# facebookresearch/habitat-lab

Hardware: AMD Instinct MI355X
Metric: env-steps/sec (SPS) PointNav RGB-D 256x256, 64 envs x 128 rollout (higher is better)
Workload: dtype f32; 1 GPU; PointNav SimpleCNN+GRU, 64 envs x 128 steps, 256x256 RGB-D synthetic; envs_per_gpu=64, rollout_steps=128, ppo_epoch=4, num_mini_batch=4, parallelism=dp1

## Files before the change

### habitat-lab_amd/csrc/gemm_ops.hip

```cpp
#include "igemm.h"
#include "igemm_dma.h"
#include "igemm_dma_wgrad.h"
#include "igemm_bf3.h"
#include "igemm_bf3_ws.h"
#include "dense_bf3.h"
#include "obs_conv_bf3.h"
#include "obs_conv_bf3_ws.h"
#include "obs_conv_patch.h"
#include "wgrad3x3_bf3.h"
#include "conv2_fwd_strip.h"
#include "conv2_dgrad_strip.h"
#include "conv3_dgrad_strip.h"
#include "obs_wgrad_bf3.h"
#include "obs_wgrad_strip.h"
#include "conv_patch_bf3.h"
#include "wgrad3x3_patch.h"
#include "prob_build.h"
#include <stdlib.h>

#include <atomic>

#include "../../include/habitat_amd.h"

namespace hab {
// ... 84 lines not shown

static bool patch3x3_wanted(const ConvDesc& d, int M) { return matrix_path_on(MP_PATCH3X3) && d.stride == 1 && d.KH == 3 && d.KW == 3 && M > 64; }
static PatchGeom patch3x3_geom(const float* in, int Hi, int Wi, int Ci, int Ho, int Wo, int off, int flip) {
    PatchGeom gq{};
    gq.in = in; gq.Hi = Hi; gq.Wi = Wi; gq.Ci = Ci; gq.Ho = Ho; gq.Wo = Wo; gq.KH = 3; gq.KW = 3;
    gq.off_h = off; gq.off_w = off; gq.flip = flip;
    return gq;
}

int conv_fwd(const ConvDesc& d, const float* x, const float* wf, const float* bias, float* y, int relu, float* ws,
             size_t ws_floats, hipStream_t stream) {
    ConvFwdProb p;
    HAB_TRY(build(p, d, x, wf, bias, y, relu));
    if (matrix_path_on(MP_CONV2_FWD | MP_RC))
        HAB_TRY_FORM(conv2_fwd_strip(p, ws, ws_floats, stream));
    if (patch3x3_wanted(d, p.M))
        HAB_TRY_FORM(conv_patch_bf3_dispatch(p, patch3x3_geom(x, d.H, d.W, d.C, p.g.Ho, p.g.Wo, -d.pad, 0), ws, ws_floats, stream));
    return run_igemm(p, ws, ws_floats, stream);
}
int64_t obs_conv_weight_image_floats() { return ((int64_t)OCP_W_ELEMS + 1) / 2 + 4; }
int obs_conv_weight_image(const float* wf, int Cout, int KH, int KW, int C, void* img, hipStream_t stream) {
    return obs_conv_patch_weight_image(wf, Cout, KH, KW, C, reinterpret_cast<unsigned short*>(img), stream);
}
int obs_conv_fwd(const ConvDesc& d, const ObsView& obs, const float* wf, const float* bias, float* y, int relu, float* ws,
                 size_t ws_floats, hipStream_t stream, const void* wimg) {
    ObsConvFwdProb p;
    HAB_TRY(build(p, d, obs, wf, bias, y, relu));
    if (matrix_path_on(MP_OBS_PATCH | MP_OBS) && p.quad)
        HAB_TRY_FORM(obs_conv_patch_launch(p, ws, ws_floats, stream, reinterpret_cast<const unsigned short*>(wimg)));
    if (matrix_path_on(MP_WS | MP_OBS) && p.quad && p.M > 64)
        HAB_TRY_FORM(obs_conv_bf3_ws_launch(p, ws, ws_floats, stream));
    if (matrix_path_on(MP_OBS) && p.quad && p.M > 64)
        HAB_TRY_FORM(obs_conv_bf3_launch<2>(p, ws, ws_floats, stream));
    return run_igemm(p, ws, ws_floats, stream);
}
__global__ void dgrad_empty_class_kernel(ConvDgradProb p) {
    const long long total = (long long)p.g.B * p.Hc * p.Wc * p.N;
    for (long long e = (long long)blockIdx.x * blockDim.x + threadIdx.x; e < total; e += (long long)gridDim.x * blockDim.x)
        p.store((int)(e / p.N), (int)(e % p.N), 0.f);
}

static int choose_conv_dgrad(const ConvDesc& d, const float* dy, const float* wd, const float* mask, const float* add, const float* dx) {
    if (!matrix_path_on(MP_CONV2_DGRAD | MP_RC)) return HAB_CONV_DGRAD_FORM_GENERAL;
    if (conv2_dgrad_strip_serves(d, dy, wd, mask, add, dx)) return HAB_CONV_DGRAD_FORM_CONV2_STRIP;
    if (conv3_dgrad_strip_serves(d, dy, wd, mask, add, dx)) return HAB_CONV_DGRAD_FORM_CONV3_STRIP;
    return HAB_CONV_DGRAD_FORM_GENERAL;
}
int conv_dgrad(const ConvDesc& d, const float* dy, const float* wd, const float* mask, const float* add, float* dx,
               float* ws, size_t ws_floats, hipStream_t stream) {
    const int form = choose_conv_dgrad(d, dy, wd, mask, add, dx);
    if (form == HAB_CONV_DGRAD_FORM_CONV2_STRIP) HAB_TRY_FORM(conv2_dgrad_strip(d, dy, wd, mask, add, dx, stream));
    if (form == HAB_CONV_DGRAD_FORM_CONV3_STRIP) HAB_TRY_FORM(conv3_dgrad_strip(d, dy, wd, mask, add, dx, stream));
// ... 271 lines not shown
    ConvDesc d;
    d.B = B; d.H = H; d.W = W; d.C = C; d.Cout = Cout; d.KH = KH; d.KW = KW; d.stride = stride; d.pad = pad;
    return d;
}
static ObsView mkobs(const uint8_t* rgb, const float* depth, const int* rows, int H, int W) {
    ObsView o;
    o.rgb = rgb; o.depth = depth; o.rows = rows; o.H = H; o.W = W; o.C = (rgb ? 3 : 0) + (depth ? 1 : 0);
    return o;
}

extern "C" int hab_conv2d_fwd(const float* x, const float* w_fwd, const float* bias, float* y, int B, int H, int W, int C,
                              int Cout, int KH, int KW, int stride, int pad, int relu, float* ws, size_t ws_floats,
                              hipStream_t stream) {
    if (!x || !w_fwd || !y) return HAB_ERR_ARG;
    return conv_fwd(mk(B, H, W, C, Cout, KH, KW, stride, pad), x, w_fwd, bias, y, relu, ws, ws_floats, stream);
}
extern "C" int hab_obs_conv2d_fwd(const uint8_t* rgb, const float* depth, const int* rows, const float* w_fwd,
                                  const float* bias, float* y, int B, int H, int W, int Cout, int KH, int KW, int stride,
                                  int pad, int relu, float* ws, size_t ws_floats, hipStream_t stream) {
    if ((!rgb && !depth) || !w_fwd || !y) return HAB_ERR_ARG;
    ObsView o = mkobs(rgb, depth, rows, H, W);
    return obs_conv_fwd(mk(B, H, W, o.C, Cout, KH, KW, stride, pad), o, w_fwd, bias, y, relu, ws, ws_floats, stream);
}
extern "C" int hab_conv2d_dgrad(const float* dy, const float* w_dgrad, const float* relu_mask, const float* add, float* dx,
                                int B, int H, int W, int C, int Cout, int KH, int KW, int stride, int pad, float* ws,
                                size_t ws_floats, hipStream_t stream) {
    if (!dy || !w_dgrad || !dx) return HAB_ERR_ARG;
    return conv_dgrad(mk(B, H, W, C, Cout, KH, KW, stride, pad), dy, w_dgrad, relu_mask, add, dx, ws, ws_floats, stream);
}
extern "C" int hab_conv2d_dgrad_form(const float* dy, const float* w_dgrad, const float* relu_mask, const float* add, float* dx,
                                     int B, int H, int W, int C, int Cout, int KH, int KW, int stride, int pad, const float* ws,
                                     size_t ws_floats) {
    (void)ws; (void)ws_floats;
    if (!dy || !w_dgrad || !dx) return HAB_ERR_ARG;
    const ConvDesc d = mk(B, H, W, C, Cout, KH, KW, stride, pad);
    const int r = check_conv(d);
    if (r != HAB_OK) return r;
    return choose_conv_dgrad(d, dy, w_dgrad, relu_mask, add, dx);
}
extern "C" int hab_conv2d_wgrad(const float* x, const float* dy, float* dw_oihw, float* dbias, int B, int H, int W, int C, int Cout,
                                int KH, int KW, int stride, int pad, float* ws, size_t ws_floats, hipStream_t stream) {
    if (!x || !dy || !dw_oihw) return HAB_ERR_ARG;
    return conv_wgrad(mk(B, H, W, C, Cout, KH, KW, stride, pad), x, dy, dw_oihw, dbias, ws, ws_floats, stream);
}
extern "C" int hab_obs_conv2d_wgrad(const uint8_t* rgb, const float* depth, const int* rows, const float* dy, float* dw_oihw,
                                    float* dbias, int B, int H, int W, int Cout, int KH, int KW, int stride, int pad, float* ws,
// ... 47 lines not shown
```

### habitat-lab_amd/csrc/obs_conv_patch.h

```cpp
#pragma once
#include <utility>

#include "igemm_bf3.h"

namespace hab {

constexpr int OCP_TH = 4;
constexpr int OCP_R = 4 * OCP_TH + 4;
constexpr int OCP_KP = 256 + 8;
constexpr int OCP_DP = 64 + 8;

constexpr int OCP_W_ELEMS = 3 * 32 * OCP_KP + 2 * 32 * OCP_DP;
__global__ void obs_patch_split_weights(const float* __restrict__ w, int N, unsigned short* __restrict__ img) {
    const int e = blockIdx.x * blockDim.x + threadIdx.x;
    if (e >= 32 * 256) return;
    const int n = e >> 8, k = e & 255, c = k & 3;
    float v = n < N ? w[(size_t)n * 256 + k] : 0.f;
    if (c < 3) v *= HAB_RCP255;
    unsigned h1, h2, h3;
    bf3_split(v, h1, h2, h3);
    img[(0 * 32 + n) * OCP_KP + k] = (unsigned short)h1;
    img[(1 * 32 + n) * OCP_KP + k] = (unsigned short)h2;
    img[(2 * 32 + n) * OCP_KP + k] = (unsigned short)h3;
    if (c == 3) {
        unsigned short* d = img + 3 * 32 * OCP_KP;
        const int kd = k >> 2;
        d[(0 * 32 + n) * OCP_DP + kd] = (unsigned short)h1;
        d[(1 * 32 + n) * OCP_DP + kd] = (unsigned short)h2;
    }
    if (k < 8) {
        img[(0 * 32 + n) * OCP_KP + 256 + k] = 0; img[(1 * 32 + n) * OCP_KP + 256 + k] = 0; img[(2 * 32 + n) * OCP_KP + 256 + k] = 0;
        unsigned short* d = img + 3 * 32 * OCP_KP;
        d[(0 * 32 + n) * OCP_DP + 64 + k] = 0; d[(1 * 32 + n) * OCP_DP + 64 + k] = 0;
    }
}

template <class F, int... Is>
__device__ __forceinline__ void ocp_static_for_impl(F& f, std::integer_sequence<int, Is...>) { (f(std::integral_constant<int, Is>()), ...); }
template <int N, class F>
__device__ __forceinline__ void ocp_static_for(F& f) { ocp_static_for_impl(f, std::make_integer_sequence<int, N>()); }

struct ObsPatchGeom {
    int W, H, Ho, Wo, tiles_per_img, ntiles;
    int units;
    int patch_elems;
};

template <int UPT>
__global__ void __launch_bounds__(512) obs_conv_patch_kernel(const ObsConvFwdProb p, const ObsPatchGeom gq, const unsigned short* __restrict__ wimg,
                                                              const int sign_schedule, const int ablate) {
    using P = ObsConvFwdProb;
    static_assert(EpiV4<P>::value, "transposed-accumulator epilogue");
    extern __shared__ __attribute__((aligned(16))) unsigned short smem16[];
    const int W = gq.W;
    const int t = threadIdx.x;
    const int lane = t & 63, wave = __builtin_amdgcn_readfirstlane(t >> 6), group = wave >> 2, gw = wave & 3, tg = t & 255;
    const int li = lane & 31, hi = lane >> 5;
    unsigned short* W12 = smem16;
    unsigned short* WD1 = W12 + 2 * 32 * OCP_KP;
    float* biasL = reinterpret_cast<float*>(WD1 + 32 * OCP_DP);
    unsigned short* P0 = WD1 + 32 * OCP_DP + 64 + group * gq.patch_elems;
    unsigned short* P1 = P0 + OCP_R * W * 4;
    unsigned short* P2 = P1 + OCP_R * W;

    for (int i = t; i < 2 * 32 * OCP_KP / 8; i += 512) reinterpret_cast<u32x4*>(W12)[i] = reinterpret_cast<const u32x4*>(wimg)[i];
    for (int i = t; i < 32 * OCP_DP / 8; i += 512) reinterpret_cast<u32x4*>(WD1)[i] = reinterpret_cast<const u32x4*>(wimg + 3 * 32 * OCP_KP)[i];
    if (t < 32) biasL[t] = (p.bias && t < p.N) ? p.bias[t] : 0.f;
    bf16x8 w3f[8][2], wd2f[4];
    {
        const unsigned short* w3 = wimg + 2 * 32 * OCP_KP + li * OCP_KP + hi * 8;
        const unsigned short* wd = wimg + 3 * 32 * OCP_KP + li * OCP_DP + hi * 8;
#pragma unroll
        for (int kh = 0; kh < 8; ++kh)
#pragma unroll
            for (int s = 0; s < 2; ++s) w3f[kh][s] = *reinterpret_cast<const bf16x8*>(w3 + kh * 32 + s * 16);
#pragma unroll
        for (int j = 0; j < 4; ++j) wd2f[j] = *reinterpret_cast<const bf16x8*>(wd + 32 * OCP_DP + j * 16);
    }

    auto tile_of = [&](int vb) {
        const int q = gq.ntiles >> 3, r = gq.ntiles & 7, xcd = vb & 7, idx = vb >> 3;
        return (xcd < r ? xcd * (q + 1) : r * (q + 1) + (xcd - r) * q) + idx;
    };

    struct Rgb12 { uint32_t d0, d1, d2; };
    Rgb12 rg[UPT];
    f32x4 dp[UPT];
    const int qpr = W >> 2;
    auto tile_base = [&](int tile, int& y0) {
        const int img = tile / gq.tiles_per_img;
        y0 = 4 * (tile - img * gq.tiles_per_img) * OCP_TH;
        return (size_t)p.obs.srow(img) * gq.H;
    };
    auto unit_pix = [&](size_t frame, int y0, int j, bool& ok) {
        const int u = tg + 256 * j;
        const int r = u / qpr, x4 = u - r * qpr;
        const int y = y0 + r;
        ok = (u < gq.units) & (y < gq.H);
        return (frame + (ok ? y : 0)) * W + 4 * (ok ? x4 : 0);
    };
    auto fetch_depth = [&](int tile) {
        if (ablate & 1) return;
        int y0;
        const size_t frame = tile_base(tile, y0);
#pragma unroll
        for (int j = 0; j < UPT; ++j) {
            bool ok;
            const size_t pix = unit_pix(frame, y0, j, ok);
            dp[j] = ld4(p.obs.depth + pix);
            if (!ok) dp[j] = zero4();
        }
    };
    auto fetch_rgb = [&](int tile) {
        if (ablate & 1) return;
        int y0;
        const size_t frame = tile_base(tile, y0);
#pragma unroll
        for (int j = 0; j < UPT; ++j) {
            bool ok;
            const size_t pix = unit_pix(frame, y0, j, ok);
            rg[j] = *reinterpret_cast<const Rgb12*>(p.obs.rgb + pix * 3);
            if (!ok) { rg[j].d0 = 0; rg[j].d1 = 0; rg[j].d2 = 0; }
        }
    };
    auto stage = [&]() {
        if (ablate & 8) return;
#pragma unroll
        for (int j = 0; j < UPT; ++j) {
            const int u = tg + 256 * j;
            if (u >= gq.units) continue;
            const unsigned d[3] = {rg[j].d0, rg[j].d1, rg[j].d2};
            unsigned f[12];
#pragma unroll
            for (int e = 0; e < 12; ++e) f[e] = __float_as_uint((float)((d[e >> 2] >> (8 * (e & 3))) & 0xffu));
            unsigned a1, a2, a3, b1, b2, b3;
            bf3_split2(dp[j][0], dp[j][1], a1, a2, a3);
            bf3_split2(dp[j][2], dp[j][3], b1, b2, b3);
            u32x4 lo, hi4;
            lo[0] = bf3_pack(f[0], f[1]);  lo[1] = bf3_pack(f[2], a1 << 16);
            lo[2] = bf3_pack(f[3], f[4]);  lo[3] = bf3_pack(f[5], a1 & 0xffff0000u);
            hi4[0] = bf3_pack(f[6], f[7]); hi4[1] = bf3_pack(f[8], b1 << 16);
            hi4[2] = bf3_pack(f[9], f[10]); hi4[3] = bf3_pack(f[11], b1 & 0xffff0000u);
            unsigned short* dst = P0 + (size_t)u * 16;
            *reinterpret_cast<u32x4*>(dst) = lo;
            *reinterpret_cast<u32x4*>(dst + 8) = hi4;
            u32x2 r1, r2;
            r1[0] = a2; r1[1] = b2; r2[0] = a3; r2[1] = b3;
            *reinterpret_cast<u32x2*>(P1 + (size_t)u * 4) = r1;
            *reinterpret_cast<u32x2*>(P2 + (size_t)u * 4) = r2;
        }
    };

    const int a_px0 = (4 * gw) * W + 4 * li;
    f32x16 acc[2];
    bf16x8 fr[2][5];
    auto load_step = [&](auto stc) {
        constexpr int st = decltype(stc)::value, set = st & 1;
        if constexpr (st < 4) {
#pragma unroll
            for (int i = 0; i < 2; ++i) {
                const int px = a_px0 + (2 * st + hi) * W + 128 * i;
                u32x4 v1, v2;
                const u32x2 l1 = *reinterpret_cast<const u32x2*>(P1 + px), h1 = *reinterpret_cast<const u32x2*>(P1 + px + 4);
                const u32x2 l2 = *reinterpret_cast<const u32x2*>(P2 + px), h2 = *reinterpret_cast<const u32x2*>(P2 + px + 4);
                v1[0] = l1[0]; v1[1] = l1[1]; v1[2] = h1[0]; v1[3] = h1[1];
                v2[0] = l2[0]; v2[1] = l2[1]; v2[2] = h2[0]; v2[3] = h2[1];
                fr[set][i] = __builtin_bit_cast(bf16x8, v1);
                fr[set][2 + i] = __builtin_bit_cast(bf16x8, v2);
            }
            fr[set][4] = *reinterpret_cast<const bf16x8*>(WD1 + li * OCP_DP + (2 * st + hi) * 8);
        } else {
            constexpr int kh = (st - 4) >> 1, s_ = (st - 4) & 1;
#pragma unroll
            for (int i = 0; i < 2; ++i)
                fr[set][i] = *reinterpret_cast<const bf16x8*>(P0 + (size_t)(a_px0 + kh * W + 128 * i) * 4 + (2 * s_ + hi) * 8);
#pragma unroll
            for (int pl = 0; pl < 2; ++pl)
                fr[set][2 + pl] = *reinterpret_cast<const bf16x8*>(W12 + (pl * 32 + li) * OCP_KP + kh * 32 + s_ * 16 + hi * 8);
        }
    };
    auto flip = [&](bf16x8 f, const unsigned sgn) {
        u32x4 v = __builtin_bit_cast(u32x4, f);
        v[0] ^= sgn; v[1] ^= sgn; v[2] ^= sgn; v[3] ^= sgn;
        return __builtin_bit_cast(bf16x8, v);
    };
    auto mma_step = [&](auto stc, const unsigned sgn) {
        constexpr int st = decltype(stc)::value, set = st & 1;
        if constexpr (st < 4) {
            const bf16x8 a1[2] = {flip(fr[set][0], sgn), flip(fr[set][1], sgn)}, a2[2] = {flip(fr[set][2], sgn), flip(fr[set][3], sgn)};
            const bf16x8 wd1 = fr[set][4];
#pragma unroll
            for (int i = 0; i < 2; ++i) acc[i] = __builtin_amdgcn_mfma_f32_32x32x16_bf16(wd1, a2[i], acc[i], 0, 0, 0);
#pragma unroll
            for (int i = 0; i < 2; ++i) acc[i] = __builtin_amdgcn_mfma_f32_32x32x16_bf16(wd2f[st], a1[i], acc[i], 0, 0, 0);
#pragma unroll
            for (int i = 0; i < 2; ++i) acc[i] = __builtin_amdgcn_mfma_f32_32x32x16_bf16(wd1, a1[i], acc[i], 0, 0, 0);
        } else {
            constexpr int kh = (st - 4) >> 1, s_ = (st - 4) & 1;
            const bf16x8 a[2] = {flip(fr[set][0], sgn), flip(fr[set][1], sgn)};
#pragma unroll
            for (int i = 0; i < 2; ++i) acc[i] = __builtin_amdgcn_mfma_f32_32x32x16_bf16(w3f[kh][s_], a[i], acc[i], 0, 0, 0);
#pragma unroll
            for (int i = 0; i < 2; ++i) acc[i] = __builtin_amdgcn_mfma_f32_32x32x16_bf16(fr[set][3], a[i], acc[i], 0, 0, 0);
#pragma unroll
            for (int i = 0; i < 2; ++i) acc[i] = __builtin_amdgcn_mfma_f32_32x32x16_bf16(fr[set][2], a[i], acc[i], 0, 0, 0);
        }
    };
    auto matrix_phase = [&](const unsigned sgn) {
#pragma unroll
        for (int i = 0; i < 2; ++i)
#pragma unroll
            for (int v = 0; v < 16; ++v) acc[i][v] = 0.0f;
        if (ablate & 2) return;
        load_step(std::integral_constant<int, 0>());
        auto body = [&](auto stc) {
            constexpr int st = decltype(stc)::value;
            if constexpr (st + 1 < 20) load_step(std::integral_constant<int, st + 1>());
            mma_step(stc, sgn);
        };
        ocp_static_for<20>(body);
    };
    auto store_tile = [&](int tile, bool neg) {
        if ((ablate & 4) && acc[0][0] != 12345.f) return;
        const int img = tile / gq.tiles_per_img, ho = (tile - img * gq.tiles_per_img) * OCP_TH + gw;
        if (ho >= gq.Ho) return;
#pragma unroll
        for (int i = 0; i < 2; ++i) {
            const int wo = 32 * i + li;
            if (wo >= gq.Wo) continue;
            const size_t base = ((size_t)(img * gq.Ho + ho) * gq.Wo + wo) * p.N;
#pragma unroll
            for (int g = 0; g < 4; ++g) {
                const int n = 8 * g + 4 * hi;
                if (n + 3 >= p.N) continue;
                f32x4 v;
                v[0] = acc[i][4 * g]; v[1] = acc[i][4 * g + 1]; v[2] = acc[i][4 * g + 2]; v[3] = acc[i][4 * g + 3];
                if (neg) { v[0] = -v[0]; v[1] = -v[1]; v[2] = -v[2]; v[3] = -v[3]; }
                v += *reinterpret_cast<const f32x4*>(biasL + n);
                if (p.relu) { v[0] = fmaxf(v[0], 0.f); v[1] = fmaxf(v[1], 0.f); v[2] = fmaxf(v[2], 0.f); v[3] = fmaxf(v[3], 0.f); }
                if (p.y) *reinterpret_cast<f32x4*>(p.y + base + n) = v;
            }
        }
    };

    const int vstep = 2 * gridDim.x;
    const int vb0 = blockIdx.x + group * gridDim.x;
    const int n_mine = vb0 < gq.ntiles ? (gq.ntiles - vb0 + vstep - 1) / vstep : 0;
    const int n_first = (int)blockIdx.x < gq.ntiles ? (gq.ntiles - (int)blockIdx.x + vstep - 1) / vstep : 0;
    if (n_first == 0) return;
    if (n_mine > 0) { fetch_depth(tile_of(vb0)); if (group == 0) fetch_rgb(tile_of(vb0)); }
    if (group == 0) stage();
    __syncthreads();
    for (int pI = 0; pI <= 2 * n_first; ++pI) {
        if ((pI & 1) == group) {
            const int k = pI >> 1;
            if (k < n_mine) {
                if (k + 1 < n_mine) fetch_depth(tile_of(vb0 + (k + 1) * vstep));
                const int tile = tile_of(vb0 + k * vstep);
                matrix_phase((sign_schedule && (tile & 1)) ? 0x80008000u : 0u);
            }
        } else {
            const int kd = (pI - 1 - group) / 2;
            const int ks = (pI + 1 - group) / 2;
            if (ks < n_mine) {
                fetch_rgb(tile_of(vb0 + ks * vstep));
                stage();
            }
            if (pI >= 1 + group && kd < n_mine) {
                const int tile_d = tile_of(vb0 + kd * vstep);
                store_tile(tile_d, sign_schedule && (tile_d & 1));
            }
        }
        __syncthreads();
    }
}

inline int obs_conv_patch_weight_image(const float* w_packed, int N, int KH, int KW, int C, unsigned short* img, hipStream_t stream) {
    if (KH != 8 || KW != 8 || C != 4 || N > 32 || (N & 3) || !w_packed || !img || (reinterpret_cast<uintptr_t>(img) & 15)) return HAB_NOT_APPLICABLE;
    obs_patch_split_weights<<<32, 256, 0, stream>>>(w_packed, N, img);
    HAB_LAUNCH_CHECK();
    return HAB_OK;
}

inline int obs_conv_patch_launch(const ObsConvFwdProb& p, float* ws, size_t ws_floats, hipStream_t stream, const unsigned short* wimg_cached = nullptr) {
    const ConvGeom& g = p.g;
    if (!p.quad || g.KH != 8 || g.KW != 8 || g.stride != 4 || g.pad != 0 || p.N > 32 || (p.N & 3) || p.K != 256 || g.W > 256 || (g.W & 3) || g.Wo > 64 ||
        g.Wo < 1 || p.M <= 0)
        return HAB_NOT_APPLICABLE;
    if (!wimg_cached && (!ws || ws_floats * 4 < (size_t)OCP_W_ELEMS * 2 || (reinterpret_cast<uintptr_t>(ws) & 15))) return HAB_NOT_APPLICABLE;
    if (reinterpret_cast<uintptr_t>(wimg_cached) & 15) return HAB_NOT_APPLICABLE;
    ObsPatchGeom gq;
    gq.W = g.W; gq.H = g.H; gq.Ho = g.Ho; gq.Wo = g.Wo;
    gq.tiles_per_img = cdiv(g.Ho, OCP_TH);
    gq.ntiles = g.B * gq.tiles_per_img;
    gq.units = OCP_R * (g.W >> 2);
    if (cdiv(gq.units, 256) > 5) return HAB_NOT_APPLICABLE;
    gq.patch_elems = OCP_R * g.W * 6 + 64;
    const size_t lds = ((size_t)2 * 32 * OCP_KP + 32 * OCP_DP + 64 + (size_t)2 * gq.patch_elems) * 2;
    if (lds > 160 * 1024) return HAB_NOT_APPLICABLE;
    const unsigned short* wimg = wimg_cached;
    if (!wimg) {
        unsigned short* built = reinterpret_cast<unsigned short*>(ws);
        obs_patch_split_weights<<<32, 256, 0, stream>>>(p.w, p.N, built);
        HAB_LAUNCH_CHECK();
        wimg = built;
    }
    auto kern = obs_conv_patch_kernel<5>;
    static const hipError_t attr_err = hipFuncSetAttribute(reinterpret_cast<const void*>(kern), hipFuncAttributeMaxDynamicSharedMemorySize, 160 * 1024);
    if (attr_err != hipSuccess) return (int)attr_err;
    const int sign_schedule = bf3_sign_schedule();
    static const int ablate = hab_env_int("HAB_OCP_ABLATE", 0);
    const int pairs = (gq.ntiles + 1) / 2;
    const int grid = pairs < 256 ? (pairs + 7) / 8 * 8 : 256;
    kern<<<grid, 512, lds, stream>>>(p, gq, wimg, sign_schedule, ablate);
    HAB_LAUNCH_CHECK();
    return HAB_OK;
}

}
```

### habitat-lab_amd/csrc/ops.h

```cpp
#pragma once
#include "hab_common.h"

namespace hab {

struct ConvDesc {
    int B, H, W, C, Cout, KH, KW, stride, pad;
    int Creal = 0;
    int Ho() const { return (H + 2 * pad - KH) / stride + 1; }
    int Wo() const { return (W + 2 * pad - KW) / stride + 1; }
};
struct ObsView;

int conv_fwd(const ConvDesc& d, const float* x, const float* wf, const float* bias, float* y, int relu, float* ws,
             size_t ws_floats, hipStream_t stream);
int obs_conv_fwd(const ConvDesc& d, const ObsView& obs, const float* wf, const float* bias, float* y, int relu, float* ws,
                 size_t ws_floats, hipStream_t stream, const void* wimg = nullptr);
int64_t obs_conv_weight_image_floats();
int obs_conv_weight_image(const float* wf, int Cout, int KH, int KW, int C, void* img, hipStream_t stream);
int conv_dgrad(const ConvDesc& d, const float* dy, const float* wd, const float* mask, const float* add, float* dx,
               float* ws, size_t ws_floats, hipStream_t stream);
int conv_wgrad(const ConvDesc& d, const float* x, const float* dy, float* dw_oihw, float* dbias, float* ws, size_t ws_floats,
               hipStream_t stream);
int obs_conv_wgrad(const ConvDesc& d, const ObsView& obs, const float* dy, float* dw_oihw, float* dbias, float* ws,
                   size_t ws_floats, hipStream_t stream);
// ... 52 lines not shown
                          int ldx0, const float* dout, float* dx0, int lddx0, const float* dx_mask, int ldmask, int mask_cols,
                          const PackInfo& pk, float* scratch , float* ws, size_t ws_floats, hipStream_t stream);
int rnn_step_layer_forward(int rnn_type, int H, const RnnLayerParams& lp, const float* x, int ldx, const float* h_in, int h_in_stride,
                           const float* c_in, int c_in_stride, const uint8_t* masks, int n, float* gi_scratch, float* h_out,
                           int h_out_stride, float* c_out, int c_out_stride, float* ws, size_t ws_floats, hipStream_t stream);
int rnn_seq_layer_backward(int rnn_type, int H, const RnnLayerParams& lp, const RnnWork& wk, const float* x, int ldx,
                           const float* dout, float* dx, int lddx, const float* dx_mask, int ldmask, int mask_cols,
                           const PackInfo& pk, float* scratch , float* ws, size_t ws_floats,
                           hipStream_t stream);
enum MatrixPath : int {
    MP_RC = 1 << 0,
    MP_OBS = 1 << 1,
    MP_IJ = 1 << 2,
    MP_IJ_WGRAD = 1 << 3,
    MP_PATCH3X3 = 1 << 4,
    MP_WS = 1 << 5,
    MP_OBS_PATCH = 1 << 6,
    MP_WGRAD_STRIP = 1 << 7,
    MP_CONV2_FWD = 1 << 8,
    MP_CONV2_DGRAD = 1 << 9,
    MP_DENSE = 1 << 10,
    MP_DENSE_ALL = 1 << 11,
    MP_RNN_STEPWISE = 1 << 12,
    MP_DEFAULT = 2047,
};
int matrix_path_bits();
inline bool matrix_path_on(int bits) { return (matrix_path_bits() & bits) == bits; }
int rnn_tm_prepare(const uint8_t* masks, const int* rows, int B, uint8_t* frame_mask, int* iota, hipStream_t stream);
int rnn_tm_layer_forward(int rnn_type, int H, const RnnLayerParams& lp, const RnnWork& wk, const float* x, int ldx, const float* hinit,
                         const float* cinit, const uint8_t* frame_mask, int n, int T_total, int t0, int t1, float* ws, size_t ws_floats,
                         hipStream_t stream);
int rnn_tm_layer_backward(int rnn_type, int H, const RnnLayerParams& lp, const RnnWork& wk, const float* dout, float* dx, int lddx,
                          const float* dx_mask, int ldmask, int mask_cols, const uint8_t* frame_mask, const int* iota, int n, int T, int t0,
                          int t1, float* scratch, float* ws, size_t ws_floats, hipStream_t stream);
int rnn_tm_layer_param_grads(int rnn_type, int H, const RnnLayerParams& lp, const RnnWork& wk, const float* x, int ldx, int P, float* ws,
                             size_t ws_floats, hipStream_t stream);

}
```

### habitat-lab_amd/habitat_amd/_lib.py

```python
from __future__ import annotations

import ctypes as C
import os
from ctypes import POINTER, c_char_p, c_double, c_float, c_int, c_int32, c_int64, c_size_t, c_uint8, c_uint32, c_void_p

_HERE = os.path.dirname(os.path.abspath(__file__))
LIB_PATH = os.path.join(_HERE, "libhabitat_amd.so")

vp = c_void_p
ALLREDUCE_FN = C.CFUNCTYPE(None, c_void_p, c_int, c_float, c_void_p)
GRAD_READY_FN = C.CFUNCTYPE(None, c_int64, c_int64, c_void_p)


class HabError(RuntimeError):
    pass


class PolicyDesc(C.Structure):
    _fields_ = [(n, c_int32) for n in (
        "arch", "backbone", "baseplanes", "normalize_visual_inputs", "rnn_type", "rnn_layers", "hidden", "num_actions",
        "H", "W", "has_rgb", "has_depth", "goal_dim", "max_frames", "max_envs", "visual_order", "has_semantic",
        "num_object_categories", "has_compass", "has_gps", "action_dist", "gauss_flags")] + [("gauss_min_std", c_float),
                                                                                                ("gauss_max_std", c_float),
                                                                                                ("pointgoal_dim", c_int32),
# ... 49 lines not shown
    "hab_obs_resize_crop": (c_int, [vp, vp, c_int, c_int, c_int, c_int, c_int, c_int, c_int, c_int, c_int, c_int, c_int, c_int, vp]),
    "hab_obs_resize_crop_form": (c_int, [vp, c_int, c_int, c_int, c_int, c_int, c_int, c_int, c_int]),
    "hab_obs_project": (c_int, [vp, c_int, vp, c_int, c_int, c_int, c_int, c_int, vp, vp, c_int, c_int, vp]),
    "hab_rollout_step_stats": (c_int, [vp, vp, vp, vp, vp, vp, vp, c_int, c_int, vp]),
    "hab_compute_returns": (c_int, [vp, vp, vp, vp, vp, c_int, c_int, c_float, c_float, c_int, c_int, vp]),
    "hab_advantages": (c_int, [vp, vp, vp, c_int, c_int, vp, vp, vp]),
    "hab_ppo_loss": (c_int, [vp, vp, vp, vp, vp, vp, vp, vp, c_int, c_float, c_float, c_float, c_int, vp, vp, vp, vp, vp]),
    "hab_ppo_loss_ver": (c_int, [vp, vp, vp, vp, vp, vp, vp, vp, c_int, c_float, c_float, c_float, c_int, vp, vp, vp, c_int64, vp, c_float,
                                 vp, vp, vp, vp, vp]),
    "hab_lagrange_adam_step": (c_int, [vp, vp, vp, vp, c_float, c_float, c_float, c_float, c_float, c_int, c_float, c_float, vp, vp]),
    "hab_ver_compute_returns": (c_int, [vp, vp, vp, vp, vp, vp, vp, vp, c_int, c_double, c_double, vp]),
    "hab_ver_is_coeffs": (c_int, [vp, c_int, c_int, c_int, vp, vp, vp]),
    "hab_clip_adam_step": (c_int, [vp, vp, vp, vp, c_size_t, vp, c_int, c_float, c_float, c_float, c_float, c_float,
                                   c_float, c_int, vp, vp]),
    "hab_sample_actions": (c_int, [vp, vp, vp, c_int, c_int, c_int, vp]),
    "hab_set_matrix_path": (c_int, [c_int]),
    "hab_conv2d_fwd": (c_int, [vp, vp, vp, vp] + [c_int] * 10 + [vp, c_size_t, vp]),
    "hab_obs_conv2d_fwd": (c_int, [vp, vp, vp, vp, vp, vp] + [c_int] * 9 + [vp, c_size_t, vp]),
    "hab_conv2d_dgrad": (c_int, [vp, vp, vp, vp, vp] + [c_int] * 9 + [vp, c_size_t, vp]),
    "hab_conv2d_wgrad": (c_int, [vp, vp, vp, vp] + [c_int] * 9 + [vp, c_size_t, vp]),
    "hab_obs_conv2d_wgrad": (c_int, [vp, vp, vp, vp, vp, vp] + [c_int] * 8 + [vp, c_size_t, vp]),
    "hab_obs_conv2d_wgrad_form": (c_int, [vp, vp, vp, vp, vp, vp] + [c_int] * 8 + [vp, c_size_t]),
    "hab_conv2d_dgrad_form": (c_int, [vp, vp, vp, vp, vp] + [c_int] * 9 + [vp, c_size_t]),
    "hab_linear_fwd": (c_int, [vp, c_int, vp, c_int, vp, vp, c_int, c_int, c_int, c_int, c_int, c_int, vp, c_size_t, vp]),
    "hab_linear_dgrad": (c_int, [vp, c_int, vp, c_int, vp, c_int, vp, c_int, c_int, c_int, c_int, c_int, vp, c_size_t, vp]),
    "hab_linear_wgrad": (c_int, [vp, c_int, vp, c_int, vp, c_int, c_int, c_int, c_int, c_int, c_int, c_int, vp, c_size_t, vp]),
    "hab_colsum": (c_int, [vp, c_int, c_int, c_int, vp, c_int, vp, c_size_t, vp]),
    "hab_repack_conv_weight": (c_int, [vp, vp, vp, c_int, c_int, c_int, c_int, c_int, vp]),
    "hab_repack_flatten_weight": (c_int, [vp, vp, c_int, c_int, c_int, vp]),
    "hab_transpose2d": (c_int, [vp, vp, c_int, c_int, vp]),
    "hab_obs_ingest_pool": (c_int, [vp, vp, vp, vp, vp, c_int, c_int, c_int, c_int, c_int, c_int, c_int, vp]),
    "hab_obs_ingest_pool_sensors": (c_int, [vp, vp, vp, vp, c_int, vp, vp, c_int, c_int, c_int, c_int, vp, vp, vp, vp, vp, vp]),
    "hab_fused_gather": (c_int, [vp, vp, c_int, vp, vp, c_int, c_int, c_int, c_int, c_int, vp]),
    "hab_channel_moments": (c_int, [vp, c_int64, c_int, c_int, vp, vp, vp, c_int, vp]),
    "hab_running_mean_var_update": (c_int, [vp, vp, vp, vp, vp, c_float, c_int, vp]),
    "hab_running_mean_var_normalize": (c_int, [vp, c_int64, c_int, c_int, vp, vp, vp]),
    "hab_groupnorm_fwd": (c_int, [vp, vp, vp, vp, vp, vp, vp, c_int, c_int, c_int, c_int, c_int, c_float, vp, c_int64, vp]),
    "hab_groupnorm_bwd": (c_int, [vp, vp, vp, vp, vp, vp, vp, vp, vp, c_int, c_int, c_int, c_int, vp, c_int64, vp]),
    "hab_split_weight_planes": (c_int, [vp, c_int, c_int, vp, vp]),
    "hab_stem_split_weights": (c_int, [vp, vp, vp]),
    "hab_stem_conv_wgrad": (c_int, [vp, vp, vp, c_int, c_int, c_int, c_int, vp, c_size_t, vp, vp]),
    "hab_stem_conv_fwd": (c_int, [vp, vp, vp, c_int, c_int, c_int, vp, vp, c_int, vp]),
    "hab_conv_gn_fwd": (c_int, [vp] * 9 + [c_int] * 11 + [c_float, vp]),
    "hab_maxpool3x3s2_fwd": (c_int, [vp, vp, vp, c_int, c_int, c_int, c_int, vp]),
    "hab_maxpool3x3s2_bwd": (c_int, [vp, vp, vp, c_int, c_int, c_int, c_int, vp]),
    "hab_nav_embed_fwd": (c_int, [POINTER(EmbedSlot), c_int, vp, vp, vp, c_int, c_int, c_int, vp, vp]),
# ... 76 lines not shown
```

### include/habitat_amd.h

```cpp
#ifndef HABITAT_AMD_H
#define HABITAT_AMD_H

#include <stddef.h>
#include <stdint.h>

#ifdef __cplusplus
extern "C" {
#endif

#ifndef __HIP_PLATFORM_AMD__
typedef struct ihipStream_t* hipStream_t;
#endif

#define HAB_ABI_VERSION 1
int hab_abi_version(void);
const char* hab_error_string(int code);

int hab_synth_step(uint8_t* rgb , float* depth , float* goal , float* reward ,
                   uint8_t* not_done , int64_t* env_t , int64_t* since_reset , uint32_t seed,
                   uint32_t env_offset, int N, int H, int W, int advance, hipStream_t stream);
int hab_synth_objectnav_sensors(int32_t* semantic, int64_t* objectgoal, float* compass, float* gps, const int64_t* env_t,
                                uint32_t seed, uint32_t env_offset, int N, int H, int W, hipStream_t stream);

#define HAB_NAV2D_STATE_BYTES 224
// ... 140 lines not shown
                           float beta2, float eps, int step, float log_alpha_min, float log_alpha_max,
                           float* alpha_out , hipStream_t stream);

int hab_ver_compute_returns(const float* rewards, const float* value_preds, const uint8_t* is_stale, float* returns,
                            const int32_t* select_inds, const int32_t* step_offsets, const int32_t* sequence_lengths,
                            const uint8_t* last_sequence_in_batch_mask, int F, double gamma, double tau, hipStream_t stream);
int hab_ver_is_coeffs(const int64_t* environment_ids, int n, int num_envs, int num_steps, int32_t* counts_scratch, float* is_coeffs,
                      hipStream_t stream);

int hab_clip_adam_step(float* params, const float* grads, float* exp_avg, float* exp_avg_sq, size_t n,
                       double* scratch_partials, int scratch_len, float grad_scale, float max_grad_norm, float lr,
                       float beta1, float beta2, float eps, int step, float* grad_norm_out, hipStream_t stream);

int hab_sample_actions(const float* probs, const float* exp_noise, int64_t* actions, int n, int A, int deterministic,
                       hipStream_t stream);

int hab_set_matrix_path(int mode);

int hab_conv2d_fwd(const float* x, const float* w_fwd, const float* bias, float* y, int B, int H, int W, int C, int Cout,
                   int KH, int KW, int stride, int pad, int relu, float* ws, size_t ws_floats, hipStream_t stream);
int hab_obs_conv2d_fwd(const uint8_t* rgb, const float* depth, const int* rows, const float* w_fwd, const float* bias,
                       float* y, int B, int H, int W, int Cout, int KH, int KW, int stride, int pad, int relu, float* ws,
                       size_t ws_floats, hipStream_t stream);
int hab_conv2d_dgrad(const float* dy, const float* w_dgrad, const float* relu_mask, const float* add, float* dx, int B,
                     int H, int W, int C, int Cout, int KH, int KW, int stride, int pad, float* ws, size_t ws_floats,
                     hipStream_t stream);
int hab_conv2d_wgrad(const float* x, const float* dy, float* dw_oihw, float* dbias, int B, int H, int W, int C, int Cout,
                     int KH, int KW, int stride, int pad, float* ws, size_t ws_floats, hipStream_t stream);
int hab_obs_conv2d_wgrad(const uint8_t* rgb, const float* depth, const int* rows, const float* dy, float* dw_oihw,
                         float* dbias, int B, int H, int W, int Cout, int KH, int KW, int stride, int pad, float* ws,
                         size_t ws_floats, hipStream_t stream);
#define HAB_OBS_WGRAD_FORM_IGEMM 0
#define HAB_OBS_WGRAD_FORM_IM2COL 1
#define HAB_OBS_WGRAD_FORM_STRIP 2
int hab_obs_conv2d_wgrad_form(const uint8_t* rgb, const float* depth, const int* rows, const float* dy, float* dw_oihw,
                              float* dbias, int B, int H, int W, int Cout, int KH, int KW, int stride, int pad, const float* ws,
                              size_t ws_floats);
#define HAB_CONV_DGRAD_FORM_GENERAL 0
#define HAB_CONV_DGRAD_FORM_CONV2_STRIP 1
#define HAB_CONV_DGRAD_FORM_CONV3_STRIP 2
int hab_conv2d_dgrad_form(const float* dy, const float* w_dgrad, const float* relu_mask, const float* add, float* dx, int B,
                          int H, int W, int C, int Cout, int KH, int KW, int stride, int pad, const float* ws, size_t ws_floats);
int hab_linear_fwd(const float* x, int ldx, const float* w, int ldw, const float* bias, float* y, int ldy, int M, int N,
                   int K, int relu, int accumulate, float* ws, size_t ws_floats, hipStream_t stream);
int hab_linear_dgrad(const float* dy, int lddy, const float* w, int ldw, const float* relu_mask, int ldmask, float* dx,
                     int lddx, int M, int n_in, int n_out, int accumulate, float* ws, size_t ws_floats,
// ... 231 lines not shown
```

Measured before the change: 65240 env-steps/s.

## Add hoisted-load variant of obs conv patch kernel using buffer loads

Adds a HOIST template variant of the observation 8x8/stride-4 conv patch kernel and makes it the default. It uses raw buffer loads with per-tile resource descriptors, so out-of-range rows return zero without per-element masking. Both groups prefetch RGB and depth for the next tile ahead of the matrix phase, the sign flip moves from the MFMA operands into the staging step, and the first MFMA step takes a zero accumulator instead of an explicit clear. The output store also uses buffer stores with a fast divider, and the old path stays reachable through a new MP_OBS_PATCH_PLAIN bit and a form query API. The early fetch raises register pressure, and the buffer descriptors rely on their size bounds for correctness.

```diff
diff --git a/habitat-lab_amd/csrc/gemm_ops.hip b/habitat-lab_amd/csrc/gemm_ops.hip
--- a/habitat-lab_amd/csrc/gemm_ops.hip
+++ b/habitat-lab_amd/csrc/gemm_ops.hip
@@ -130,12 +130,18 @@
 int obs_conv_weight_image(const float* wf, int Cout, int KH, int KW, int C, void* img, hipStream_t stream) {
     return obs_conv_patch_weight_image(wf, Cout, KH, KW, C, reinterpret_cast<unsigned short*>(img), stream);
 }
+static int choose_obs_fwd(const ObsConvFwdProb& p, const float* ws, size_t ws_floats, const void* wimg) {
+    if (!(matrix_path_on(MP_OBS_PATCH | MP_OBS) && obs_conv_patch_covers(p, ws, ws_floats, reinterpret_cast<const unsigned short*>(wimg))))
+        return HAB_OBS_FWD_FORM_OTHER;
+    return matrix_path_on(MP_OBS_PATCH_PLAIN) ? HAB_OBS_FWD_FORM_PATCH_PLAIN : HAB_OBS_FWD_FORM_PATCH;
+}
 int obs_conv_fwd(const ConvDesc& d, const ObsView& obs, const float* wf, const float* bias, float* y, int relu, float* ws,
                  size_t ws_floats, hipStream_t stream, const void* wimg) {
     ObsConvFwdProb p;
     HAB_TRY(build(p, d, obs, wf, bias, y, relu));
-    if (matrix_path_on(MP_OBS_PATCH | MP_OBS) && p.quad)
-        HAB_TRY_FORM(obs_conv_patch_launch(p, ws, ws_floats, stream, reinterpret_cast<const unsigned short*>(wimg)));
+    const int form = choose_obs_fwd(p, ws, ws_floats, wimg);
+    if (form != HAB_OBS_FWD_FORM_OTHER)
+        HAB_TRY_FORM(obs_conv_patch_launch(p, ws, ws_floats, stream, reinterpret_cast<const unsigned short*>(wimg), form == HAB_OBS_FWD_FORM_PATCH));
     if (matrix_path_on(MP_WS | MP_OBS) && p.quad && p.M > 64)
         HAB_TRY_FORM(obs_conv_bf3_ws_launch(p, ws, ws_floats, stream));
     if (matrix_path_on(MP_OBS) && p.quad && p.M > 64)
@@ -453,6 +459,16 @@
     ObsView o = mkobs(rgb, depth, rows, H, W);
     return obs_conv_fwd(mk(B, H, W, o.C, Cout, KH, KW, stride, pad), o, w_fwd, bias, y, relu, ws, ws_floats, stream);
 }
+extern "C" int hab_obs_conv2d_fwd_form(const uint8_t* rgb, const float* depth, const int* rows, const float* w_fwd,
+                                       const float* bias, float* y, int B, int H, int W, int Cout, int KH, int KW, int stride,
+                                       int pad, int relu, const float* ws, size_t ws_floats) {
+    if ((!rgb && !depth) || !w_fwd || !y) return HAB_ERR_ARG;
+    ObsView o = mkobs(rgb, depth, rows, H, W);
+    ObsConvFwdProb p;
+    const int r = build(p, mk(B, H, W, o.C, Cout, KH, KW, stride, pad), o, w_fwd, bias, y, relu);
+    if (r != HAB_OK) return r;
+    return choose_obs_fwd(p, ws, ws_floats, nullptr);
+}
 extern "C" int hab_conv2d_dgrad(const float* dy, const float* w_dgrad, const float* relu_mask, const float* add, float* dx,
                                 int B, int H, int W, int C, int Cout, int KH, int KW, int stride, int pad, float* ws,
                                 size_t ws_floats, hipStream_t stream) {
diff --git a/habitat-lab_amd/csrc/obs_conv_patch.h b/habitat-lab_amd/csrc/obs_conv_patch.h
--- a/habitat-lab_amd/csrc/obs_conv_patch.h
+++ b/habitat-lab_amd/csrc/obs_conv_patch.h
@@ -4,6 +4,8 @@
 #include "igemm_bf3.h"
 
 namespace hab {
+
+typedef unsigned int u32x3 __attribute__((ext_vector_type(3)));
 
 constexpr int OCP_TH = 4;
 constexpr int OCP_R = 4 * OCP_TH + 4;
@@ -42,11 +44,12 @@
 
 struct ObsPatchGeom {
     int W, H, Ho, Wo, tiles_per_img, ntiles;
+    FastDiv dTpi;
     int units;
     int patch_elems;
 };
 
-template <int UPT>
+template <int UPT, bool HOIST>
 __global__ void __launch_bounds__(512) obs_conv_patch_kernel(const ObsConvFwdProb p, const ObsPatchGeom gq, const unsigned short* __restrict__ wimg,
                                                               const int sign_schedule, const int ablate) {
     using P = ObsConvFwdProb;
@@ -87,6 +90,21 @@
     Rgb12 rg[UPT];
     f32x4 dp[UPT];
     const int qpr = W >> 2;
+    struct TileRows { size_t first; int rows; };
+    auto tile_rows = [&](int tile, bool want) {
+        TileRows tr{0, 0};
+        if (HOIST && want && !(ablate & 1)) {
+            const int img = gq.dTpi.div(tile);
+            const int y0 = 4 * (tile - img * gq.tiles_per_img) * OCP_TH;
+            tr.first = (size_t)p.obs.srow(img) * gq.H + y0;
+            tr.rows = gq.H - y0 < OCP_R ? gq.H - y0 : OCP_R;
+        }
+        return tr;
+    };
+    auto tile_rsrc = [&](const TileRows& tr, const void* base, int bpp) {
+        const uint8_t* first = reinterpret_cast<const uint8_t*>(base) + tr.first * W * bpp;
+        return __builtin_amdgcn_make_buffer_rsrc(const_cast<uint8_t*>(first), 0, tr.rows * W * bpp, 0x00020000);
+    };
     auto tile_base = [&](int tile, int& y0) {
         const int img = tile / gq.tiles_per_img;
         y0 = 4 * (tile - img * gq.tiles_per_img) * OCP_TH;
@@ -99,7 +117,13 @@
         ok = (u < gq.units) & (y < gq.H);
         return (frame + (ok ? y : 0)) * W + 4 * (ok ? x4 : 0);
     };
-    auto fetch_depth = [&](int tile) {
+    auto fetch_depth = [&](int tile, const TileRows& tr) {
+        if constexpr (HOIST) {
+            const __amdgpu_buffer_rsrc_t rd = tile_rsrc(tr, p.obs.depth, 4);
+#pragma unroll
+            for (int j = 0; j < UPT; ++j) dp[j] = __builtin_bit_cast(f32x4, __builtin_amdgcn_raw_buffer_load_b128(rd, 16 * tg + 4096 * j, 0, 0));
+            return;
+        }
         if (ablate & 1) return;
         int y0;
         const size_t frame = tile_base(tile, y0);
@@ -111,7 +135,16 @@
             if (!ok) dp[j] = zero4();
         }
     };
-    auto fetch_rgb = [&](int tile) {
+    auto fetch_rgb = [&](int tile, const TileRows& tr) {
+        if constexpr (HOIST) {
+            const __amdgpu_buffer_rsrc_t rr = tile_rsrc(tr, p.obs.rgb, 3);
+#pragma unroll
+            for (int j = 0; j < UPT; ++j) {
+                const u32x3 v = __builtin_amdgcn_raw_buffer_load_b96(rr, 12 * tg + 3072 * j, 0, 0);
+                rg[j].d0 = v[0]; rg[j].d1 = v[1]; rg[j].d2 = v[2];
+            }
+            return;
+        }
         if (ablate & 1) return;
         int y0;
         const size_t frame = tile_base(tile, y0);
@@ -123,7 +156,7 @@
             if (!ok) { rg[j].d0 = 0; rg[j].d1 = 0; rg[j].d2 = 0; }
         }
     };
-    auto stage = [&]() {
+    auto stage = [&](const unsigned sgn) {
         if (ablate & 8) return;
 #pragma unroll
         for (int j = 0; j < UPT; ++j) {
@@ -141,11 +174,13 @@
             lo[2] = bf3_pack(f[3], f[4]);  lo[3] = bf3_pack(f[5], a1 & 0xffff0000u);
             hi4[0] = bf3_pack(f[6], f[7]); hi4[1] = bf3_pack(f[8], b1 << 16);
             hi4[2] = bf3_pack(f[9], f[10]); hi4[3] = bf3_pack(f[11], b1 & 0xffff0000u);
+            if constexpr (HOIST) { lo ^= sgn; hi4 ^= sgn; }
             unsigned short* dst = P0 + (size_t)u * 16;
             *reinterpret_cast<u32x4*>(dst) = lo;
             *reinterpret_cast<u32x4*>(dst + 8) = hi4;
             u32x2 r1, r2;
             r1[0] = a2; r1[1] = b2; r2[0] = a3; r2[1] = b3;
+            if constexpr (HOIST) { r1 ^= sgn; r2 ^= sgn; }
             *reinterpret_cast<u32x2*>(P1 + (size_t)u * 4) = r1;
             *reinterpret_cast<u32x2*>(P2 + (size_t)u * 4) = r2;
         }
@@ -153,6 +188,7 @@
 
     const int a_px0 = (4 * gw) * W + 4 * li;
     f32x16 acc[2];
+    if constexpr (HOIST) { acc[0] = f32x16(0.f); acc[1] = f32x16(0.f); }
     bf16x8 fr[2][5];
     auto load_step = [&](auto stc) {
         constexpr int st = decltype(stc)::value, set = st & 1;
@@ -180,6 +216,7 @@
         }
     };
     auto flip = [&](bf16x8 f, const unsigned sgn) {
+        if constexpr (HOIST) return f;
         u32x4 v = __builtin_bit_cast(u32x4, f);
         v[0] ^= sgn; v[1] ^= sgn; v[2] ^= sgn; v[3] ^= sgn;
         return __builtin_bit_cast(bf16x8, v);
@@ -190,7 +227,7 @@
             const bf16x8 a1[2] = {flip(fr[set][0], sgn), flip(fr[set][1], sgn)}, a2[2] = {flip(fr[set][2], sgn), flip(fr[set][3], sgn)};
             const bf16x8 wd1 = fr[set][4];
 #pragma unroll
-            for (int i = 0; i < 2; ++i) acc[i] = __builtin_amdgcn_mfma_f32_32x32x16_bf16(wd1, a2[i], acc[i], 0, 0, 0);
+            for (int i = 0; i < 2; ++i) acc[i] = __builtin_amdgcn_mfma_f32_32x32x16_bf16(wd1, a2[i], (HOIST && st == 0) ? f32x16(0.f) : acc[i], 0, 0, 0);
 #pragma unroll
             for (int i = 0; i < 2; ++i) acc[i] = __builtin_amdgcn_mfma_f32_32x32x16_bf16(wd2f[st], a1[i], acc[i], 0, 0, 0);
 #pragma unroll
@@ -207,10 +244,12 @@
         }
     };
     auto matrix_phase = [&](const unsigned sgn) {
-#pragma unroll
-        for (int i = 0; i < 2; ++i)
-#pragma unroll
-            for (int v = 0; v < 16; ++v) acc[i][v] = 0.0f;
+        if constexpr (!HOIST) {
+#pragma unroll
+            for (int i = 0; i < 2; ++i)
+#pragma unroll
+                for (int v = 0; v < 16; ++v) acc[i][v] = 0.0f;
+        }
         if (ablate & 2) return;
         load_step(std::integral_constant<int, 0>());
         auto body = [&](auto stc) {
@@ -220,8 +259,32 @@
         };
         ocp_static_for<20>(body);
     };
+    const unsigned y_lane = (unsigned)(li * p.N + 4 * hi);
     auto store_tile = [&](int tile, bool neg) {
         if ((ablate & 4) && acc[0][0] != 12345.f) return;
+        if constexpr (HOIST) {
+            const int img = gq.dTpi.div(tile), ho = (tile - img * gq.tiles_per_img) * OCP_TH + gw;
+            if (ho >= gq.Ho) return;
+            if (!p.y) return;
+            const __amdgpu_buffer_rsrc_t ry = __builtin_amdgcn_make_buffer_rsrc(p.y + (size_t)(img * gq.Ho + ho) * gq.Wo * p.N, 0, gq.Wo * p.N * 4, 0x00020000);
+            const unsigned smask = neg ? 0x80000000u : 0u;
+#pragma unroll
+            for (int i = 0; i < 2; ++i) {
+                if (32 * i + li >= gq.Wo) continue;
+#pragma unroll
+                for (int g = 0; g < 4; ++g) {
+                    if (8 * g + 4 * hi + 3 >= p.N) continue;
+                    u32x4 b;
+                    b[0] = __float_as_uint(acc[i][4 * g]); b[1] = __float_as_uint(acc[i][4 * g + 1]);
+                    b[2] = __float_as_uint(acc[i][4 * g + 2]); b[3] = __float_as_uint(acc[i][4 * g + 3]);
+                    b ^= smask;
+                    f32x4 v = __builtin_bit_cast(f32x4, b) + *reinterpret_cast<const f32x4*>(biasL + 8 * g + 4 * hi);
+                    if (p.relu) { v[0] = fmaxf(v[0], 0.f); v[1] = fmaxf(v[1], 0.f); v[2] = fmaxf(v[2], 0.f); v[3] = fmaxf(v[3], 0.f); }
+                    __builtin_amdgcn_raw_buffer_store_b128(__builtin_bit_cast(u32x4, v), ry, (int)(4 * (y_lane + (unsigned)(32 * i * p.N + 8 * g))), 0, 0);
+                }
+            }
+            return;
+        }
         const int img = tile / gq.tiles_per_img, ho = (tile - img * gq.tiles_per_img) * OCP_TH + gw;
         if (ho >= gq.Ho) return;
 #pragma unroll
@@ -248,23 +311,32 @@
     const int n_mine = vb0 < gq.ntiles ? (gq.ntiles - vb0 + vstep - 1) / vstep : 0;
     const int n_first = (int)blockIdx.x < gq.ntiles ? (gq.ntiles - (int)blockIdx.x + vstep - 1) / vstep : 0;
     if (n_first == 0) return;
-    if (n_mine > 0) { fetch_depth(tile_of(vb0)); if (group == 0) fetch_rgb(tile_of(vb0)); }
-    if (group == 0) stage();
+    if (n_mine > 0) {
+        const TileRows tr = tile_rows(tile_of(vb0), true);
+        fetch_depth(tile_of(vb0), tr);
+        if (group == 0 || HOIST) fetch_rgb(tile_of(vb0), tr);
+    }
+    const auto tile_sign = [&](int tile) { return (sign_schedule && (tile & 1)) ? 0x80008000u : 0u; };
+    if (group == 0 && n_mine > 0) stage(tile_sign(tile_of(vb0)));
     __syncthreads();
     for (int pI = 0; pI <= 2 * n_first; ++pI) {
         if ((pI & 1) == group) {
             const int k = pI >> 1;
             if (k < n_mine) {
-                if (k + 1 < n_mine) fetch_depth(tile_of(vb0 + (k + 1) * vstep));
+                const int tile_n = tile_of(vb0 + (k + 1) * vstep);
+                const TileRows tr = tile_rows(tile_n, k + 1 < n_mine);
+                if (HOIST || k + 1 < n_mine) fetch_depth(tile_n, tr);
+                if constexpr (HOIST) fetch_rgb(tile_n, tr);
                 const int tile = tile_of(vb0 + k * vstep);
-                matrix_phase((sign_schedule && (tile & 1)) ? 0x80008000u : 0u);
+                matrix_phase(tile_sign(tile));
             }
         } else {
             const int kd = (pI - 1 - group) / 2;
             const int ks = (pI + 1 - group) / 2;
             if (ks < n_mine) {
-                fetch_rgb(tile_of(vb0 + ks * vstep));
-                stage();
+                const int tile_s = tile_of(vb0 + ks * vstep);
+                if constexpr (!HOIST) fetch_rgb(tile_s, tile_rows(tile_s, true));
+                stage(tile_sign(tile_s));
             }
             if (pI >= 1 + group && kd < n_mine) {
                 const int tile_d = tile_of(vb0 + kd * vstep);
@@ -282,32 +354,32 @@
     return HAB_OK;
 }
 
-inline int obs_conv_patch_launch(const ObsConvFwdProb& p, float* ws, size_t ws_floats, hipStream_t stream, const unsigned short* wimg_cached = nullptr) {
+inline bool obs_conv_patch_covers(const ObsConvFwdProb& p, const float* ws, size_t ws_floats, const unsigned short* wimg_cached, ObsPatchGeom* gq_out = nullptr) {
     const ConvGeom& g = p.g;
     if (!p.quad || g.KH != 8 || g.KW != 8 || g.stride != 4 || g.pad != 0 || p.N > 32 || (p.N & 3) || p.K != 256 || g.W > 256 || (g.W & 3) || g.Wo > 64 ||
         g.Wo < 1 || p.M <= 0)
-        return HAB_NOT_APPLICABLE;
-    if (!wimg_cached && (!ws || ws_floats * 4 < (size_t)OCP_W_ELEMS * 2 || (reinterpret_cast<uintptr_t>(ws) & 15))) return HAB_NOT_APPLICABLE;
-    if (reinterpret_cast<uintptr_t>(wimg_cached) & 15) return HAB_NOT_APPLICABLE;
+        return false;
+    if (!wimg_cached && (!ws || ws_floats * 4 < (size_t)OCP_W_ELEMS * 2 || (reinterpret_cast<uintptr_t>(ws) & 15))) return false;
+    if (reinterpret_cast<uintptr_t>(wimg_cached) & 15) return false;
     ObsPatchGeom gq;
     gq.W = g.W; gq.H = g.H; gq.Ho = g.Ho; gq.Wo = g.Wo;
     gq.tiles_per_img = cdiv(g.Ho, OCP_TH);
+    gq.dTpi = FastDiv(gq.tiles_per_img);
     gq.ntiles = g.B * gq.tiles_per_img;
     gq.units = OCP_R * (g.W >> 2);
-    if (cdiv(gq.units, 256) > 5) return HAB_NOT_APPLICABLE;
+    if (cdiv(gq.units, 256) > 5) return false;
     gq.patch_elems = OCP_R * g.W * 6 + 64;
-    const size_t lds = ((size_t)2 * 32 * OCP_KP + 32 * OCP_DP + 64 + (size_t)2 * gq.patch_elems) * 2;
-    if (lds > 160 * 1024) return HAB_NOT_APPLICABLE;
-    const unsigned short* wimg = wimg_cached;
-    if (!wimg) {
-        unsigned short* built = reinterpret_cast<unsigned short*>(ws);
-        obs_patch_split_weights<<<32, 256, 0, stream>>>(p.w, p.N, built);
-        HAB_LAUNCH_CHECK();
-        wimg = built;
-    }
-    auto kern = obs_conv_patch_kernel<5>;
+    if (((size_t)2 * 32 * OCP_KP + 32 * OCP_DP + 64 + (size_t)2 * gq.patch_elems) * 2 > 160 * 1024) return false;
+    if (gq_out) *gq_out = gq;
+    return true;
+}
+
+template <bool HOIST>
+inline int obs_conv_patch_launch_form(const ObsConvFwdProb& p, const ObsPatchGeom& gq, const unsigned short* wimg, hipStream_t stream) {
+    auto kern = obs_conv_patch_kernel<5, HOIST>;
     static const hipError_t attr_err = hipFuncSetAttribute(reinterpret_cast<const void*>(kern), hipFuncAttributeMaxDynamicSharedMemorySize, 160 * 1024);
     if (attr_err != hipSuccess) return (int)attr_err;
+    const size_t lds = ((size_t)2 * 32 * OCP_KP + 32 * OCP_DP + 64 + (size_t)2 * gq.patch_elems) * 2;
     const int sign_schedule = bf3_sign_schedule();
     static const int ablate = hab_env_int("HAB_OCP_ABLATE", 0);
     const int pairs = (gq.ntiles + 1) / 2;
@@ -317,4 +389,18 @@
     return HAB_OK;
 }
 
-}
+inline int obs_conv_patch_launch(const ObsConvFwdProb& p, float* ws, size_t ws_floats, hipStream_t stream, const unsigned short* wimg_cached = nullptr,
+                                 bool hoist = true) {
+    ObsPatchGeom gq;
+    if (!obs_conv_patch_covers(p, ws, ws_floats, wimg_cached, &gq)) return HAB_NOT_APPLICABLE;
+    const unsigned short* wimg = wimg_cached;
+    if (!wimg) {
+        unsigned short* built = reinterpret_cast<unsigned short*>(ws);
+        obs_patch_split_weights<<<32, 256, 0, stream>>>(p.w, p.N, built);
+        HAB_LAUNCH_CHECK();
+        wimg = built;
+    }
+    return hoist ? obs_conv_patch_launch_form<true>(p, gq, wimg, stream) : obs_conv_patch_launch_form<false>(p, gq, wimg, stream);
+}
+
+}
diff --git a/habitat-lab_amd/csrc/ops.h b/habitat-lab_amd/csrc/ops.h
--- a/habitat-lab_amd/csrc/ops.h
+++ b/habitat-lab_amd/csrc/ops.h
@@ -98,6 +98,7 @@
     MP_DENSE = 1 << 10,
     MP_DENSE_ALL = 1 << 11,
     MP_RNN_STEPWISE = 1 << 12,
+    MP_OBS_PATCH_PLAIN = 1 << 13,
     MP_DEFAULT = 2047,
 };
 int matrix_path_bits();
diff --git a/habitat-lab_amd/habitat_amd/_lib.py b/habitat-lab_amd/habitat_amd/_lib.py
--- a/habitat-lab_amd/habitat_amd/_lib.py
+++ b/habitat-lab_amd/habitat_amd/_lib.py
@@ -95,6 +95,7 @@
     "hab_obs_conv2d_wgrad": (c_int, [vp, vp, vp, vp, vp, vp] + [c_int] * 8 + [vp, c_size_t, vp]),
     "hab_obs_conv2d_wgrad_form": (c_int, [vp, vp, vp, vp, vp, vp] + [c_int] * 8 + [vp, c_size_t]),
     "hab_conv2d_dgrad_form": (c_int, [vp, vp, vp, vp, vp] + [c_int] * 9 + [vp, c_size_t]),
+    "hab_obs_conv2d_fwd_form": (c_int, [vp, vp, vp, vp, vp, vp] + [c_int] * 9 + [vp, c_size_t]),
     "hab_linear_fwd": (c_int, [vp, c_int, vp, c_int, vp, vp, c_int, c_int, c_int, c_int, c_int, c_int, vp, c_size_t, vp]),
     "hab_linear_dgrad": (c_int, [vp, c_int, vp, c_int, vp, c_int, vp, c_int, c_int, c_int, c_int, c_int, vp, c_size_t, vp]),
     "hab_linear_wgrad": (c_int, [vp, c_int, vp, c_int, vp, c_int, c_int, c_int, c_int, c_int, c_int, c_int, vp, c_size_t, vp]),
diff --git a/include/habitat_amd.h b/include/habitat_amd.h
--- a/include/habitat_amd.h
+++ b/include/habitat_amd.h
@@ -186,6 +186,12 @@
 int hab_obs_conv2d_fwd(const uint8_t* rgb, const float* depth, const int* rows, const float* w_fwd, const float* bias,
                        float* y, int B, int H, int W, int Cout, int KH, int KW, int stride, int pad, int relu, float* ws,
                        size_t ws_floats, hipStream_t stream);
+#define HAB_OBS_FWD_FORM_OTHER 0
+#define HAB_OBS_FWD_FORM_PATCH 1
+#define HAB_OBS_FWD_FORM_PATCH_PLAIN 2
+int hab_obs_conv2d_fwd_form(const uint8_t* rgb, const float* depth, const int* rows, const float* w_fwd, const float* bias,
+                            float* y, int B, int H, int W, int Cout, int KH, int KW, int stride, int pad, int relu, const float* ws,
+                            size_t ws_floats);
 int hab_conv2d_dgrad(const float* dy, const float* w_dgrad, const float* relu_mask, const float* add, float* dx, int B,
                      int H, int W, int C, int Cout, int KH, int KW, int stride, int pad, float* ws, size_t ws_floats,
                      hipStream_t stream);
```

Result: faster. 66920 env-steps/s (median of 6 runs) (+2.6%).
